# satoken/ractip

Hardware: AMD Instinct MI355X
Metric: sequence-pairs/sec (incl. bp+hp+ap DP; host strings in, thresholded matrices out) at n=500 (higher is better)
Workload: dtype f64; 1 GPU; synthetic random pairs n=500/500, std::mt19937(12345) stream (BASELINE config 3); scoring=CONTRAfold complementary (708 weights)

## Files before the change

### ractip_amd/csrc/compute.hip

```cpp
#include <hip/hip_runtime.h>

#include <algorithm>
#include <cmath>
#include <cstring>
#include <string>
#include <vector>

#include "ctx.h"
#include "kernels.h"

namespace rh::host {

template <class L, class... Args>
int run_graphed(rh_ctx* c, GraphSlot& g, hipStream_t stream, int k, L launcher, const Args&... args)
{
    const auto launch = [&] { int rc = RH_OK; ((rc = rc ? rc : launcher(c, args)), ...); return rc; };
    if (!c->use_graphs || c->time_cls >= 0) return launch();
    size_t key = 1469598103934665603ull + (sizeof(Args) + ...);
    const auto mix = [&](const void* p, size_t n) { for (size_t q = 0; q < n; q++) key = (key ^ ((const unsigned char*)p)[q]) * 0x100000001b3ull; };
    (mix(&args, sizeof(Args)), ...);
    int *launch_counter = &c->n_launch[k], *far_counter = &c->n_far[k];
    if (!g.exec || g.key != key) {
        if (g.exec) { HIP_TRY(c, hipGraphExecDestroy(g.exec)); g.exec = nullptr; }
        hipGraph_t graph = nullptr;
        const int before = *launch_counter, far_before = *far_counter;
        HIP_TRY(c, hipStreamBeginCapture(stream, hipStreamCaptureModeThreadLocal));
        const int rc = launch();
        hipError_t e = hipStreamEndCapture(stream, &graph);
        if (rc) { if (graph) (void)hipGraphDestroy(graph); return rc; }
        if (e != hipSuccess) { if (graph) (void)hipGraphDestroy(graph); return fail(c, RH_ERR_HIP, "graph capture failed: %s", hipGetErrorString(e)); }
        e = hipGraphInstantiate(&g.exec, graph, nullptr, nullptr, 0);
        (void)hipGraphDestroy(graph);
        if (e != hipSuccess) { g.exec = nullptr; return fail(c, RH_ERR_HIP, "hipGraphInstantiate failed: %s", hipGetErrorString(e)); }
        g.key = key;
        g.launches = *launch_counter - before;
        g.far = *far_counter - far_before;
        *launch_counter = before;
        *far_counter = far_before;
    }
    HIP_TRY(c, hipGraphLaunch(g.exec, stream));
    *launch_counter += g.launches;
    *far_counter += g.far;
    return RH_OK;
}

McLinArgs mc_lin_args(const rh_ctx* c, int phase, const McBatch& B, const LinSet* lin, bool routed)
{
    McLinArgs A;
    A.B = B; A.lin = lin; A.phase = phase;
    A.logz = c->d_mclogz.as<double>(); A.bad = c->d_bad.as<int>();
    A.plan = plan_mc_lin(c, phase, B.nmax);
    if (routed && (!c->small_list.empty() || c->n_short > 0)) {
        A.routed = 1;
        A.small_list = c->d_small_list.as<const int>(); A.n_small = (int)c->small_list.size();
        A.n_sweep = c->d_n_sweep.as<const int>(); A.nmax_sweep = c->nmax_sweep;
        A.n_short = c->d_n_short.as<const int>(); A.nmax_short = c->nmax_short; A.short_count = c->n_short;
        A.plan_sweep = plan_mc_lin(c, phase, A.nmax_sweep);
        A.plan_short = plan_mc_lin(c, phase, A.nmax_short);
    }
    A.pin = xcd_pin(B.ns);
    A.strip_xcd = c->strip_xcd;
    A.f5_jlo = 32;
    A.f5_pass = c->f5_pass && f5_pass_lds(B.ld, 1) <= 64 * 1024;
    return A;
}

static McVlinArgs mc_vlin_args(const rh_ctx* c, int phase, bool co)
{
    McVlinArgs A;
    A.B = co ? c->co : c->mc; A.phase = phase; A.co = co;
    A.pin = xcd_pin(A.B.ns);
    A.plan = plan_mc_vlin(c, phase, co, A.B.nmax);
    A.d_vlin = c->d_vlin; A.h_vlin = c->h_vlin; A.hplen = c->h_hplen.data(); A.d_hplen = c->d_hplen.as<const double>();
    A.bad = co ? c->d_cobad.as<int>() : c->d_bad.as<int>();
    if (co) {
        const DxBatch& D = c->dx;
        if (A.B.seeded) { A.from = c->mc; A.pair_seq = c->d_pidx.as<const int>(); }
        A.hp = D.hp; A.hp_logz = D.logz; A.hp_stride = D.tab_stride; A.hp_ldd = D.ldd; A.n1max = D.n1max; A.n2max = D.n2max;
        A.cut_min = c->co_cut_min; A.cut_max = c->co_cut_max;
        A.window = c->co_window && c->co_cut_min >= 1 && (phase == 1 || A.B.seeded);
    } else {
        A.logz = c->d_mclogz.as<double>(); A.gaps = c->d_gaps.as<double>(); A.max_w = c->max_w;
        A.acc_wide = c->acc_wide && (size_t)VM_COUNT * A.B.tab_stride * sizeof(double) < ((size_t)1 << 32);
        A.acc_final_t = c->acc_final_t && c->max_w <= 15;
    }
    return A;
}

static DxLinArgs dx_args(const rh_ctx* c)
{
    DxLinArgs A;
    A.X = c->dxl; A.plan = c->plan[2]; A.lz_chunks = c->lz_chunks;
    A.zpart = c->d_zpart.as<double>(); A.zbar = c->d_zbar.as<double>();
    A.logz = c->d_logz.as<double>(); A.bad = c->d_dxbad.as<int>();
    return A;
}

DxLinArgs dx_lin_args(const rh_ctx* c)
{
    DxLinArgs A = dx_args(c);
    A.dm = c->d_dxlin; A.hm = &c->h_dxlin;
    return A;
}

static DxLinArgs dx_vlin_args(const rh_ctx* c)
{
    DxLinArgs A = dx_args(c);
    A.vdx_s = c->vdx_s; A.sem20 = c->vienna_sem == kViennaSem20;
    return A;
}

int flagged(rh_ctx* c, const int* d_flags, int n, hipStream_t st, std::vector<int>* set)
{
    std::vector<int> flags(n);
    HIP_TRY(c, hipMemcpyAsync(flags.data(), d_flags, sizeof(int) * n, hipMemcpyDeviceToHost, st));
    HIP_TRY(c, hipStreamSynchronize(st));
    set->clear();
    for (int k = 0; k < n; k++) if (flags[k]) set->push_back(k);
    return RH_OK;
}

struct Attempt {
    bool defer_log = false;
    bool deferred = false;
    std::vector<int> flagged_seqs;
    std::vector<int> flagged_pairs;
    bool went_log = false;
    Ev outside_from = kEvMcInside;
};

static int close_dx_phase(rh_ctx* c)
{
    HIP_TRY(c, hipEventRecord(c->ev[kEvDxEnd], c->s_dx));
    if (!c->overlap) HIP_TRY(c, hipStreamSynchronize(c->s_dx));
    return RH_OK;
}

template <class Launch>
static int restart_mc_log(rh_ctx* c, Launch launch)
{
    c->n_launch[0] = c->n_launch[1] = 0;
    c->n_far[0] = c->n_far[1] = 0;
    HIP_TRY(c, hipEventRecord(c->ev[kEvMcStart], c->s_mc));
    HIP_TRY(c, hipMemsetAsync(c->d_bp.p, 0, sizeof(double) * c->mc.tri_stride * c->mc.ns, c->s_mc));
    if (int rc = launch()) return rc;
    if (c->last_path == 0) c->last_path = 2;
// ... 280 lines not shown
```

### ractip_amd/csrc/ctx.h

```cpp
#pragma once
#include <hip/hip_runtime.h>

#include <cassert>
#include <cstdint>
#include <cstring>
#include <string>
#include <type_traits>
#include <vector>

#include "../../include/ractip_hot.h"
#include "batch.h"
#include "score_model.h"
#include "lin_model.h"
#include "vienna_model.h"
#include "scale_order.h"

struct rh_ctx;

namespace rh::host {

struct DevBuf {
    void* p = nullptr;
    size_t cap = 0;
    DevBuf() = default;
// ... 248 lines not shown
    McBatch co = {};
    DevBuf d_coseq;
    DevBuf d_con;
    DevBuf d_cotab;
    DevBuf d_cof5;
    DevBuf d_cobp;
    DevBuf d_cobad;
    double ms[4] = {0, 0, 0, 0};
    int n_launch[3] = {0, 0, 0};
    int n_far[3] = {0, 0, 0};
    bool overlap = true;
    int time_cls = -1;
    std::vector<hipEvent_t> tev;
    size_t tev_n = 0;
    Ctx() = default;
    Ctx(const Ctx&) = delete;
    ~Ctx() { delete[] lin_r; delete h_score; delete h_vienna; }
};

}

struct rh_ctx : rh::host::Ctx {};

#define HIP_TRY(c, call)                                                                         \
    do {                                                                                         \
        hipError_t e_ = (call);                                                                  \
        if (e_ != hipSuccess)                                                                    \
            return fail(c, e_ == hipErrorOutOfMemory ? RH_ERR_OOM : RH_ERR_HIP, "%s failed: %s", \
                        #call, hipGetErrorString(e_));                                           \
    } while (0)

#define KLAUNCH(c, cls, kern, grid, block, stream, ...)                                                   \
    do {                                                                                                  \
        const bool timed_ = (c)->time_cls == (cls) && (c)->tev_n + 2 <= (c)->tev.size();                  \
        if (timed_) (void)hipEventRecord((c)->tev[(c)->tev_n++], stream);                                 \
        hipLaunchKernelGGL(kern, grid, block, 0, stream, __VA_ARGS__);                                    \
        if (timed_) (void)hipEventRecord((c)->tev[(c)->tev_n++], stream);                                 \
    } while (0)

namespace rh::host {

inline size_t tri_size(int n) { return (size_t)(n + 1) * (n + 2) / 2; }

int fail(rh_ctx* c, int code, const char* fmt, ...);
int ensure(rh_ctx* c, DevBuf& buf, size_t bytes, bool zero);
int stage(rh_ctx* c, int ns, const char* const* seqs, const int* lens, bool with_mc, bool with_dx, const char* const* cons = nullptr,
          const char* const* co_cons = nullptr, int npairs = 0, const int* first = nullptr, const int* second = nullptr);
inline int seq_of(const Ctx* c, int p, int side) { return c->pair_seq[2 * (size_t)p + side]; }
inline void pairs_of_seq(const Ctx* c, int k, std::vector<int>* pairs)
{
    for (int p = 0; p < c->np; p++)
        if (seq_of(c, p, 0) == k || seq_of(c, p, 1) == k) pairs->push_back(p);
}
template <class K> struct Named { K kern; const char* name; };
#define NAMED(...) {__VA_ARGS__, #__VA_ARGS__}
template <class Row, size_t N, class Pred>
const Row& row_of(const Row (&rows)[N], Pred&& is)
{
    for (const Row& r : rows) if (is(r)) return r;
    assert(!"the plan names a kernel combination that has no row");
    return rows[0];
}
inline int xcd_pin(int ns) { return ns % 8 == 0 ? 1 : 0; }
inline dim3 seq_grid(int pin, int ns, int groups) { return pin ? dim3(ns, groups) : dim3(groups, ns); }
struct SweepPass {
    rh_ctx* c;
    const SweepPlan& P;
    const McBatch& B;
    hipStream_t st;
    int k;
    int far2_next = -1;
    int last_block() const { return P.BS > 0 ? (B.nmax - 1) / P.BS : 0; }
};
int launch_mc_log(rh_ctx* c, int pin, const McBatch& B, double* logz_out);
SweepPlan plan_mc_lin(const rh_ctx* c, int phase, int nmax);
int launch_mc_lin(rh_ctx* c, const McLinArgs& A);
void far_products(const rh_ctx* c, int phase, int nmax, bool mfma, SweepPlan* P);
const char* far_name(SweepPlan::Far far, int BS, int phase);
void far_inside_after(const SweepPass& S, int done);
void far_outside_begin(SweepPass& S, int top);
void far_outside_before(SweepPass& S, int d);
std::vector<double> strip_weights(const LinModel& L, bool* ok_out = nullptr);
size_t f5_pass_lds(int ld, int phase);
int launch_mc_vienna(rh_ctx* c, int pin);
SweepPlan plan_mc_vlin(const rh_ctx* c, int phase, bool co, int nmax);
int launch_mc_vlin(rh_ctx* c, const McVlinArgs& A);
int launch_cofold(rh_ctx* c);
int select_vlin(rh_ctx* c, int model);
extern const double kVRungS[Ctx::kVRungs];
int launch_dx_log(rh_ctx* c, const DxBatch& D);
SweepPlan plan_dx_lin(const rh_ctx* c, int w);
SweepPlan plan_dx_vlin(bool sem20);
int launch_dx_lin(rh_ctx* c, const DxLinArgs& A);
int launch_dx_vlin(rh_ctx* c, const DxLinArgs& A);
int launch_dx_vlog(rh_ctx* c);
int retry_mc_lin_rungs(rh_ctx* c, int first_model, std::vector<int>* rest, int (&rescued_by)[Ctx::kRungs + 1]);
int recompute_mc_subset_log(rh_ctx* c, const std::vector<int>& F);
int retry_dx_lin_rungs(rh_ctx* c, std::vector<int>* rest);
int recompute_dx_subset_log(rh_ctx* c, const std::vector<int>& F);
int recompute_pairs_on_helper(rh_ctx* c, const std::vector<int>& P);
int compute(rh_ctx* c);
McLinArgs mc_lin_args(const rh_ctx* c, int phase, const McBatch& B, const LinSet* lin, bool routed);
DxLinArgs dx_lin_args(const rh_ctx* c);
int flagged(rh_ctx* c, const int* d_flags, int n, hipStream_t st, std::vector<int>* set);

}

rh_ctx* make_ctx_for_helper(int device, int model, const char* param_file, const char* defaults_file, int use_bl, int semantics);
```

### ractip_amd/csrc/launch_contrafold.hip

```cpp
#include <hip/hip_runtime.h>

#include <algorithm>
#include <cmath>
#include <cstring>
#include <string>
#include <vector>

#include "ctx.h"
#include "kernels.h"

__global__ void log_finish(rh::McBatch B, double* __restrict__ logz)
{
    const int sq = blockIdx.x * blockDim.x + threadIdx.x;
    if (sq < B.ns) logz[sq] = B.f5i[(size_t)sq * B.ld + B.n[sq]];
}

namespace rh::host {

int launch_mc_log(rh_ctx* c, int pin, const McBatch& B, double* logz_out)
{
    hipLaunchKernelGGL(mc_init, dim3((B.ns + 63) / 64), dim3(64), 0, c->s_mc, B);
    for (int d = 0; d <= B.nmax - 1; d++) {
        const int waves = std::max(B.nmax - 1 - d, 0) + 1;
        KLAUNCH(c, 0, mc_inside_diag, pin ? dim3(B.ns, (waves + 3) / 4) : dim3((waves + 3) / 4, B.ns), dim3(256), c->s_mc, B, c->d_model, d, pin);
        c->n_launch[0]++;
    }
    HIP_TRY(c, hipEventRecord(c->ev[kEvMcInside], c->s_mc));
    for (int d = B.nmax - 2; d >= 0; d--) {
        const int waves = (B.nmax - 1 - d) + 1;
        KLAUNCH(c, 2, mc_outside_diag, pin ? dim3(B.ns, (waves + 3) / 4) : dim3((waves + 3) / 4, B.ns), dim3(256), c->s_mc, B, c->d_model, d, pin);
        c->n_launch[1]++;
    }
    hipLaunchKernelGGL(log_finish, dim3((B.ns + 63) / 64), dim3(64), 0, c->s_mc, B, logz_out);
    hipLaunchKernelGGL(mc_unpaired, dim3((B.nmax + 63) / 64, B.ns), dim3(256), 0, c->s_mc, B);
    return RH_OK;
}

using InsideDiagK = void (*)(McBatch, const LinModel*, int, double, int);
struct DiagKernels { int W, BS; Named<InsideDiagK> in; Named<decltype(&lin_outside_diag<4, 16>)> out; };
#define DIAG(W, BS) {W, BS, NAMED(lin_inside_diag<W, BS, 0>), NAMED(lin_outside_diag<W, BS>)}
const DiagKernels kDiag[] = {DIAG(8, 0), DIAG(16, 0), DIAG(4, 16), DIAG(8, 16), DIAG(16, 16), DIAG(8, 32), DIAG(16, 32)};
const Named<InsideDiagK> kInsidePair = NAMED(lin_inside_diag<4, 16, 3>);
const Named<InsideDiagK> kInsideAhead[2] = {NAMED(lin_inside_diag<4, 16, 1>), NAMED(lin_inside_diag<4, 16, 2>)};
struct PairKernels { int W; Named<decltype(&lin_outside_pair<4, 16>)> out; };
const PairKernels kOutsidePair[] = {{4, NAMED(lin_outside_pair<4, 16>)}, {8, NAMED(lin_outside_pair<8, 16>)}};
struct StripKernels { int W, filt; Named<decltype(&lin_inside_strip<8, 4, 0>)> in; Named<decltype(&lin_outside_strip<8, 4, 0>)> out; };
#define STRIP(W, FILT) {W, FILT, NAMED(lin_inside_strip<8, W, FILT>), NAMED(lin_outside_strip<8, W, FILT>)}
const StripKernels kStrip[] = {STRIP(4, 0), STRIP(8, 1), STRIP(8, 0)};
struct LdsKernels { int BS; Named<decltype(&lin_far_inside<16>)> in, out; };
const LdsKernels kLds[] = {{16, NAMED(lin_far_inside<16>), NAMED(lin_far_outside<16>)}, {32, NAMED(lin_far_inside<32>), NAMED(lin_far_outside<32>)}};
const Named<decltype(&lin_far_inside_mfma)> kFarGather[2] = {NAMED(lin_far_inside_mfma), NAMED(lin_far_outside_mfma)};
const Named<decltype(&lin_far_inside_pk)> kFarPacked[2] = {NAMED(lin_far_inside_pk), NAMED(lin_far_outside_pk)};
#undef DIAG
#undef STRIP
static const DiagKernels& diag_kernels(int W, int BS) { return row_of(kDiag, [&](const DiagKernels& r) { return r.W == W && r.BS == BS; }); }
static const PairKernels& pair_kernels(int W) { return row_of(kOutsidePair, [&](const PairKernels& r) { return r.W == W; }); }
static const StripKernels& strip_kernels(int W, int filt) { return row_of(kStrip, [&](const StripKernels& r) { return r.W == W && r.filt == filt; }); }
static const LdsKernels& lds_kernels(int BS) { return row_of(kLds, [&](const LdsKernels& r) { return r.BS == BS; }); }

const char* far_name(SweepPlan::Far far, int BS, int phase)
{
    switch (far) {
        case SweepPlan::kFarLds: return phase == 0 ? lds_kernels(BS).in.name : lds_kernels(BS).out.name;
        case SweepPlan::kFarGather: return kFarGather[phase].name;
        case SweepPlan::kFarPacked: return kFarPacked[phase].name;
        default: return "";
    }
}
void far_products(const rh_ctx* c, int phase, int nmax, bool mfma, SweepPlan* P)
{
    const int from = c->far2 >= 0 ? (c->far2 ? 1 : 0) : 384;
    P->far = P->BS == 0 ? SweepPlan::kFarNone : !mfma ? SweepPlan::kFarLds : c->far_pk ? SweepPlan::kFarPacked : SweepPlan::kFarGather;
    P->far2_from = P->far == SweepPlan::kFarPacked && from > 0 && nmax >= from ? from : 0;
    P->far_name = far_name(P->far, P->BS, phase);
}

void far_inside_after(const SweepPass& S, int done)
{
    rh_ctx* c = S.c;
    const McBatch& B = S.B;
    const int D = S.P.BS ? done / S.P.BS + 1 : 0, last_block = S.last_block(), l2 = S.P.far2_from;
    if (S.P.BS == 0 || done % S.P.BS != 0 || D < 4 || D > last_block) return;
    if (S.P.far == SweepPlan::kFarLds) KLAUNCH(c, 1, (lds_kernels(S.P.BS).in.kern), dim3(last_block - D + 1, B.ns), dim3(256), S.st, B, D);
    else if (S.P.far == SweepPlan::kFarGather) KLAUNCH(c, 1, (kFarGather[0].kern), dim3(last_block - D + 1, B.ns), dim3(256), S.st, B, D);
    else {
        KLAUNCH(c, 1, lin_pack_tiles<0>, dim3(B.nb - (D - 2), B.ns, 2), dim3(256), S.st, B, D - 2, 0, (int)S.P.banded);
        if (l2 && (D + 3) % 4 == 0) {
            const int D2 = (D + 3) / 4, last2 = (B.nmax - 1) / 64;
            if (D2 >= 4 && D2 <= last2) KLAUNCH(c, 1, lin_far2_inside, dim3(last2 - D2 + 1, B.ns), dim3(256), S.st, B, D2, l2);
        }
        KLAUNCH(c, 1, (kFarPacked[0].kern), dim3(last_block - D + 1, B.ns), dim3(256), S.st, B, D, l2);
// ... 1 lines not shown
    c->n_launch[S.k]++;
    c->n_far[S.k]++;
}
void far_outside_before(SweepPass& S, int d)
{
    rh_ctx* c = S.c;
    const McBatch& B = S.B;
    const int D = S.P.BS ? (d + 1) / S.P.BS - 1 : 0, last_block = S.last_block(), l2 = S.P.far2_from;
    if (S.P.BS == 0 || (d + 1) % S.P.BS != 0 || D < 0 || D > last_block) return;
    if (S.P.far == SweepPlan::kFarLds) KLAUNCH(c, 3, (lds_kernels(S.P.BS).out.kern), dim3(last_block - D + 1, B.ns, 2), dim3(256), S.st, B, D);
    else if (S.P.far == SweepPlan::kFarGather) KLAUNCH(c, 3, (kFarGather[1].kern), dim3(last_block - D + 1, B.ns, 2), dim3(256), S.st, B, D);
    else {
        if (D + 2 <= last_block) KLAUNCH(c, 3, lin_pack_tiles<1>, dim3(B.nb - (D + 2), B.ns, 1), dim3(256), S.st, B, D + 2, 1, 0);
        if (l2) {
            const int last2 = (B.nmax - 1) / 64;
            for (; S.far2_next >= 0 && 4 * S.far2_next + 3 >= D; S.far2_next--)
                KLAUNCH(c, 3, lin_far2_outside, dim3(last2 - S.far2_next + 1, B.ns, 2), dim3(256), S.st, B, S.far2_next, l2);
        }
        KLAUNCH(c, 3, (kFarPacked[1].kern), dim3(last_block - D + 1, B.ns, 2), dim3(256), S.st, B, D, l2);
    }
    c->n_launch[S.k]++;
    c->n_far[S.k]++;
}
void far_outside_begin(SweepPass& S, int top)
{
    if (S.P.BS == 0) return;
    rh_ctx* c = S.c;
    const McBatch& B = S.B;
    const int last_block = S.last_block(), banded = S.P.banded;
    if (S.P.far == SweepPlan::kFarPacked) {
        S.far2_next = (B.nmax - 1) / 64;
        if (S.P.repack2 && last_block - 1 > 2) KLAUNCH(c, 3, lin_pack_tiles<1>, dim3(B.nb - 2, B.ns, 2), dim3(256), S.st, B, 2, 0, banded);
        for (int Dblk = std::max(2, last_block - 1); Dblk <= last_block; Dblk++)
            KLAUNCH(c, 3, lin_pack_tiles<1>, dim3(B.nb - Dblk, B.ns, 2), dim3(256), S.st, B, Dblk, 0, banded);
    }
    for (int d = (last_block + 1) * S.P.BS - 1; d > top; d -= S.P.BS) far_outside_before(S, d);
}

SweepPlan plan_mc_lin(const rh_ctx* c, int phase, int nmax)
{
    SweepPlan P;
    const int w = phase == 0 ? c->lin_w_in : c->lin_w;
    P.BS = c->lin_bs == 0 || c->lin_bs == 32 ? c->lin_bs : 16;
    P.W = w == 16 ? 16 : (w == 4 && P.BS == 16 ? 4 : 8);
    const bool all_orgs = P.W == 4 && P.BS == 16, strips_ok = c->far_pk && c->far_mfma && c->lin_bs == 16 && nmax >= kStripMinN;
    const bool strips_on = (c->strip & (phase == 0 ? 1 : 2)) && strips_ok, strips = all_orgs && strips_on;
    const StripKernels& strip = strip_kernels(c->strip_w, c->strip_w == 8 && c->strip_filt && c->strip_filt_ok);
    const DiagKernels& diag = diag_kernels(P.W, P.BS);
    bool mfma = P.BS == 16 && c->far_mfma;
    P.org = SweepPlan::kDiagonals;
    P.fine = phase == 0 ? diag.in.name : diag.out.name;
    if (strips) {
        P.org = SweepPlan::kStrips;
        P.W = strip.W;
        P.filt = strip.filt;
    } else if (phase == 0 && all_orgs && c->lookahead == 2) {
        P.org = SweepPlan::kPairs;
        P.fine = kInsidePair.name;
        mfma = true;
    } else if (phase == 0 && all_orgs && c->lookahead) {
        P.org = SweepPlan::kLookahead;
        P.fine = kInsideAhead[0].name;
    } else if (phase == 1 && mfma && (P.W == 4 || P.W == 8) && c->lookahead == 2) {
        P.org = SweepPlan::kPairs;
        P.fine = pair_kernels(P.W).out.name;
    }
    far_products(c, phase, nmax, mfma, &P);
    P.banded = strips;
    P.repack2 = phase == 1 && strips != (all_orgs && (c->strip & 1) && strips_ok);
    if (strips_on) P.fine = phase == 0 ? strip.in.name : strip.out.name;
    if (phase == 0 && P.org == SweepPlan::kPairs && !c->far_mfma) { P.fine = diag.in.name; P.far_name = far_name(SweepPlan::kFarLds, 16, 0); }
    return P;
}

static void inside_pairs(const SweepPass& S, const McLinArgs& A, int last)
{
    for (int d = 0; d <= last; d += 2) {
        const int groups = (std::max(S.B.nmax - 1 - d, 0) + 62) / 63 + 1;
        KLAUNCH(S.c, 0, (kInsidePair.kern), seq_grid(A.pin, S.B.ns, groups), dim3(256), S.st, S.B, A.lin->d, d, std::exp(-A.lin->h.s * d), A.pin);
        S.c->n_launch[0]++;
        far_inside_after(S, d + 2);
    }
}
size_t f5_pass_lds(int ld, int phase) { return sizeof(double) * ((size_t)ld + 8 + (phase ? (size_t)((ld + 255) / 256) * 256 : 0)); }

static void inside_strips(const SweepPass& S, const McLinArgs& A)
{
    rh_ctx* c = S.c;
    const McBatch& B = S.B;
    constexpr int KD = 8, GS = 64 - (KD - 1);
    const auto strip = strip_kernels(S.P.W, S.P.filt).in.kern;
    inside_pairs(S, A, 30);
    for (int d0 = 32; d0 <= B.nmax - 2; d0 += KD) {
        const int groups = (B.nmax - 1 - d0 + GS - 1) / GS;
        KLAUNCH(c, 0, strip, seq_grid(A.pin, B.ns, groups), dim3(64 * S.P.W), S.st, B, A.lin->d, A.lin->wT, d0, std::exp(-A.lin->h.s * d0),
                (A.pin && A.strip_xcd) ? 2 : A.pin);
        c->n_launch[0]++;
        far_inside_after(S, d0 + KD);
    }
    if (A.f5_pass) hipLaunchKernelGGL(lin_f5i_pass, dim3(B.ns), dim3(256), f5_pass_lds(B.ld, 0), S.st, B, A.lin->d, A.f5_jlo);
    else hipLaunchKernelGGL(lin_f5i_tail, dim3(B.ns), dim3(256), 0, S.st, B, A.lin->d, A.f5_jlo);
}
static void inside_diagonals(const SweepPass& S, const McLinArgs& A, bool ahead)
{
    const InsideDiagK full = diag_kernels(S.P.W, S.P.BS).in.kern;
    for (int d = 0; d <= S.B.nmax - 1; d++) {
        const int groups = (std::max(S.B.nmax - 1 - d, 0) + 63) / 64 + 1;
        const bool odd = ahead && (d & 1);
        KLAUNCH(S.c, 0, (!ahead ? full : kInsideAhead[odd].kern), seq_grid(A.pin, S.B.ns, groups), dim3(odd ? 64 : 64 * S.P.W), S.st, S.B, A.lin->d, d,
                std::exp(-A.lin->h.s * d), A.pin);
        S.c->n_launch[0]++;
        far_inside_after(S, d + 1);
    }
}

static void outside_strips(SweepPass& S, const McLinArgs& A)
{
    rh_ctx* c = S.c;
    const McBatch& B = S.B;
    constexpr int KD = 8, GS = 64 - (KD - 1);
    const auto strip = strip_kernels(S.P.W, S.P.filt).out.kern;
    const int d0_top = (B.nmax - 2) | (KD - 1);
    far_outside_begin(S, d0_top);
    if (A.f5_pass) hipLaunchKernelGGL(lin_f5o_pass, dim3(B.ns), dim3(256), f5_pass_lds(B.ld, 1), S.st, B, A.lin->d);
    else hipLaunchKernelGGL(lin_f5o_head, dim3(B.ns), dim3(256), 0, S.st, B, A.lin->d, B.nmax - 1, 1);
    for (int d0 = d0_top; d0 >= KD - 1; d0 -= KD) {
        far_outside_before(S, d0);
        const int groups = (B.nmax - 1 - (d0 - (KD - 1)) + GS - 1) / GS;
        KLAUNCH(c, 2, strip, seq_grid(A.pin, B.ns, groups), dim3(64 * S.P.W), S.st, B, A.lin->d, A.lin->wT, d0, (A.pin && A.strip_xcd) ? 2 : A.pin, A.bad);
        c->n_launch[1]++;
    }
}
static void outside_pairs(SweepPass& S, const McLinArgs& A)
{
    const auto pair = pair_kernels(S.P.W).out.kern;
    far_outside_begin(S, S.B.nmax - 2);
    for (int d = (S.B.nmax - 2) | 1; d >= 0; d -= 2) {
        for (int r = d; r >= d - 1 && r >= 0; r--) far_outside_before(S, r);
        const int ncol = S.B.nmax - 1 - d + 1;
        const int groups = std::max(1, (ncol - 1 + 62) / 63) + 1;
        KLAUNCH(S.c, 2, pair, seq_grid(A.pin, S.B.ns, groups), dim3(64 * S.P.W), S.st, S.B, A.lin->d, d, d, A.pin, A.bad);
        S.c->n_launch[1]++;
    }
}
static void outside_diagonals(SweepPass& S, const McLinArgs& A)
{
    const auto diag = diag_kernels(S.P.W, S.P.BS).out.kern;
    far_outside_begin(S, S.B.nmax - 2);
    for (int d = S.B.nmax - 2; d >= 0; d--) {
        far_outside_before(S, d);
        const int groups = (S.B.nmax - 1 - d + 63) / 64 + 1;
        KLAUNCH(S.c, 2, diag, seq_grid(A.pin, S.B.ns, groups), dim3(64 * S.P.W), S.st, S.B, A.lin->d, d, A.pin, A.bad);
        S.c->n_launch[1]++;
    }
}

int launch_mc_lin(rh_ctx* c, const McLinArgs& A)
{
    const McBatch& BR = A.B;
    const int phase = A.phase;
    const auto sweep = [&](const McBatch& B, const SweepPlan& Q) {
        SweepPass S{c, Q, B, c->s_mc, phase};
        if (Q.org == SweepPlan::kStrips) return phase == 0 ? inside_strips(S, A) : outside_strips(S, A);
        if (Q.org == SweepPlan::kPairs) return phase == 0 ? inside_pairs(S, A, B.nmax) : outside_pairs(S, A);
        return phase == 0 ? inside_diagonals(S, A, Q.org == SweepPlan::kLookahead) : outside_diagonals(S, A);
    };
    if (phase == 0) {
// ... 70 lines not shown
```

### ractip_amd/csrc/mccaskill_strip.hip

```cpp
#include <hip/hip_runtime.h>

#include <type_traits>
#include <utility>

#include "batch.h"
#include "dev_util.h"
#include "lin_model.h"
#include "kernels.h"

namespace rh {

namespace {

template <int V> using IC = std::integral_constant<int, V>;
template <class F, int... Is> __device__ __forceinline__ void static_for_impl(F&& f, std::integer_sequence<int, Is...>) { (f(IC<Is>{}), ...); }
template <int N, class F> __device__ __forceinline__ void static_for(F&& f) { static_for_impl(f, std::make_integer_sequence<int, N>{}); }

}

#ifdef RH_STAMPS
__device__ unsigned long long g_stamps[16];
#define RH_STAMP(k) do { const unsigned long long t_ = __builtin_amdgcn_s_memtime(); st_acc_[k] += t_ - t_prev_; t_prev_ = t_; \
        if ((k) == 8 && threadIdx.x == 0) { for (int k_ = 0; k_ < 15; k_++) if (st_acc_[k_]) atomicAdd(&g_stamps[k_], st_acc_[k_]); atomicAdd(&g_stamps[15], 1ull); } } while (0)
#define RH_STAMP_BEGIN() unsigned long long st_acc_[15] = {}; unsigned long long t_prev_ = __builtin_amdgcn_s_memtime()
extern "C" int rh_debug_stamps(unsigned long long* out, int reset)
{
    if (hipMemcpyFromSymbol(out, HIP_SYMBOL(g_stamps), sizeof(g_stamps)) != hipSuccess) return -1;
    if (reset) { unsigned long long z[16] = {}; if (hipMemcpyToSymbol(HIP_SYMBOL(g_stamps), z, sizeof(z)) != hipSuccess) return -1; }
    return 0;
}
__device__ unsigned long long g_trace[5 * 16384];
extern "C" int rh_debug_trace(unsigned long long* out)
{
    return hipMemcpyFromSymbol(out, HIP_SYMBOL(g_trace), sizeof(g_trace)) == hipSuccess ? 0 : -1;
}
#if RH_STAMPS == 3
#define RH_TRACE(slot) do { if (threadIdx.x == 0 && d0 == 256) { const unsigned lin_ = blockIdx.x + blockIdx.y * gridDim.x; if (lin_ < 16384) g_trace[5 * lin_ + (slot)] = __builtin_amdgcn_s_memrealtime(); } } while (0)
#define RH_TRACE_ID() do { if (threadIdx.x == 0 && d0 == 256) { const unsigned lin_ = blockIdx.x + blockIdx.y * gridDim.x; if (lin_ < 16384) g_trace[5 * lin_] = ((unsigned long long)__builtin_amdgcn_s_getreg((20 << 0) | (0 << 6) | (31 << 11)) << 32) | __builtin_amdgcn_s_getreg((4 << 0) | (0 << 6) | (31 << 11)); } } while (0)
#endif
#define RH_NOSTAMP(k) do { } while (0)
#define RH_NOSTAMP_BEGIN() do { } while (0)
#if RH_STAMPS == 3
#define RH_STAMPO(k) RH_NOSTAMP(k)
#define RH_STAMPO_BEGIN() RH_NOSTAMP_BEGIN()
#define RH_STAMPI(k) RH_NOSTAMP(k)
#define RH_STAMPI_BEGIN() RH_NOSTAMP_BEGIN()
#elif RH_STAMPS == 2
#define RH_STAMPO(k) RH_STAMP(k)
#define RH_STAMPO_BEGIN() RH_STAMP_BEGIN()
#define RH_STAMPI(k) RH_NOSTAMP(k)
#define RH_STAMPI_BEGIN() RH_NOSTAMP_BEGIN()
#else
#define RH_STAMPI(k) RH_STAMP(k)
#define RH_STAMPI_BEGIN() RH_STAMP_BEGIN()
#define RH_STAMPO(k) RH_NOSTAMP(k)
#define RH_STAMPO_BEGIN() RH_NOSTAMP_BEGIN()
#endif
#else
#define RH_STAMPI(k) do { } while (0)
#define RH_STAMPI_BEGIN() do { } while (0)
#define RH_STAMPO(k) do { } while (0)
#define RH_STAMPO_BEGIN() do { } while (0)
#endif
#ifndef RH_TRACE
#define RH_TRACE(slot) do { } while (0)
#define RH_TRACE_ID() do { } while (0)
#endif

template <int U, bool OUTSIDE, int CE>
__device__ __forceinline__ void filt_factored(lds_vp xb, lds_vp fw, const double* __restrict__ F, double (&g)[4])
{
    auto X = [&](int row_off, int m, int l1) -> double { return OUTSIDE ? xb[row_off + 31 + m - l1] : xb[row_off + 3 - m + l1]; };
    constexpr int par = (U + 1) & 1;
    double bw[15];
#pragma unroll
    for (int j = 0; j < 15; j++) bw[j] = F[160 + 16 * par + j];
    static_for<8>([&](auto QC) {
        constexpr int q = decltype(QC)::value, t0 = U - 1 + 4 * q, ro = q * 4 * CE;
        if constexpr (t0 + 6 >= 2 && t0 <= 30) {
            double S = 0.0, xc = 0.0;
            if constexpr (t0 >= 3) {
                double S2 = 0.0;
                static_for<t0 - 1>([&](auto LC) {
                    constexpr int l1 = decltype(LC)::value + 1, dist = (2 * l1 - t0) < 0 ? (t0 - 2 * l1) : (2 * l1 - t0);
                    if constexpr (2 * l1 != t0) {
                        const double x = X(ro, 0, l1);
                        if constexpr (l1 & 1) S = fma(bw[dist / 2], x, S); else S2 = fma(bw[dist / 2], x, S2);
                    }
                });
// ... 468 lines not shown
        fm2s[SL] = fm2; gs[SL] += g0 + g1;
    };
    auto fin = [&](auto KC) {
        constexpr int K = decltype(KC)::value, SL = K / W;
        const int d = d0 + K;
        const bool v = i <= n - 1 - d;
        double fm2 = fm2s[SL];
        const double g = gs[SL];
        if constexpr (K >= 1) {
            fm2 = fma(f1[0], SFM[(K - 1) * CS + lane + 1], fm2);
            if (1 <= d - 32) fm2 = fma(SFM1[(K - 1) * CS + lane], LDm[lane + K], fm2);
        }
        double x01 = p_x01, x10 = p_x10, x11 = p_x11, o_fc = p_fc, o_fca = p_fca, o_fm1 = p_fm1, o_fm = p_fm;
        if constexpr (K >= 3) { x01 = SFCX[(K - 3) * CS + lane + 1]; x10 = SFCX[(K - 3) * CS + lane + 2]; }
        if constexpr (K >= 4) x11 = SFCX[(K - 4) * CS + lane + 2];
        if constexpr (K >= 2) { o_fc = SFC[(K - 2) * CS + lane + 1]; o_fca = SFCA[(K - 2) * CS + lane + 1]; }
        if constexpr (K >= 1) { o_fm1 = SFM1[(K - 1) * CS + lane + 1]; o_fm = SFM[(K - 1) * CS + lane]; }
        double lk = lam_d0;
#pragma unroll
        for (int q = 0; q < K; q++) lk *= lam;
        const double hp = lk * hp30;
        const double sp = p_c01[SL] * x01 + p_c10[SL] * x10 + p_c11[SL] * x11;
        double fc = p_tjb[SL] * (g + sp + hp) + p_cst[SL] * o_fc + fm2 * p_ctja[SL];
        double fm1v = o_fca * w_mp2 + o_fm1 * w_mu;
        double fmv = fm2 + o_fm * w_mu + fm1v;
        if (!v) { fc = 0.0; fm1v = 0.0; fmv = 0.0; }
        const double fcxv = fc * p_cbx[SL], fcav = fc * p_cba[SL];
        SFM[K * CS + lane] = fmv; SFM1[K * CS + lane] = fm1v; SFCX[K * CS + lane] = fcxv; SFC[K * CS + lane] = fc; SFCA[K * CS + lane] = fcav;
    };
    RH_STAMPI(6);
#define RH_SLOT(T)                                                                                  \
    if constexpr (T < KD) {                                                                         \
        if (w == T % W) fin(IC<T>{});                                                               \
        if constexpr (T >= 1 && T + 1 < KD)                                                         \
            static_for<KD>([&](auto KC) {                                                           \
                constexpr int K = decltype(KC)::value;                                              \
                if constexpr (K > T) { if (w == K % W) addrow(IC<(T >= 1 ? T - 1 : 0)>{}, KC); }    \
            });                                                                                     \
        if constexpr (T + 1 < KD) lds_barrier();                                                    \
    }
    RH_SLOT(0) RH_SLOT(1) RH_SLOT(2) RH_SLOT(3) RH_SLOT(4) RH_SLOT(5) RH_SLOT(6) RH_SLOT(7)
#undef RH_SLOT
    RH_STAMPI(7);
    lds_barrier();
    if (lane < GS) {
#pragma unroll 1
        for (int r = w; r < 5 * KD; r += W) {
            const int tb = r / KD, k = r - tb * KD, d = d0 + k;
            const int slot_of[5] = {L_FM, L_FM1, L_FCX, L_FC, L_FCA};
            if (i <= n - 1 - d) tab[slot_of[tb] * ts + (size_t)d * ld + i] = SFM[r * CS + lane];
        }
    }
    RH_STAMPI(8);
    RH_TRACE(4);
}

__device__ __forceinline__ double f5_term(double f5, double fca, double acc) { return fma(f5, fca, acc); }
__device__ __forceinline__ double f5_entry(double prev, double r0, double r1, double r2, double r3, double w_eu, double w_ep2)
{
    return fma(prev, w_eu, (r0 + r1 + r2 + r3) * w_ep2);
}

__global__ __launch_bounds__(256) void lin_f5i_tail(McBatch B, const LinModel* __restrict__ L, int jlo)
{
    __shared__ double red[4];
    const int sq = blockIdx.x;
    if (sq >= B.ns) return;
    const int n = B.n[sq], ld = B.ld;
    const int w = threadIdx.x >> 6, lane = threadIdx.x & 63;
    double* __restrict__ f5i = B.f5i + (size_t)sq * ld;
    const double* __restrict__ fca = B.tab + (size_t)sq * B.seq_stride + L_FCA * B.tab_stride;
#pragma unroll 1
    for (int jj = jlo < 1 ? 1 : jlo; jj <= n; jj++) {
        double acc = 0.0;
        for (int k = threadIdx.x; k <= jj - 2; k += 256) acc = f5_term(f5i[k], fca[(size_t)(jj - 2 - k) * ld + (k + 1)], acc);
        acc = wsum(acc);
        if (lane == 0) red[w] = acc;
        __syncthreads();
        if (threadIdx.x == 0) f5i[jj] = f5_entry(f5i[jj - 1], red[0], red[1], red[2], red[3], L->w_eu, L->w_ep2);
        __syncthreads();
    }
}

constexpr int kF5Blk = 16;

__global__ __launch_bounds__(256) void lin_f5i_pass(McBatch B, const LinModel* __restrict__ L, int jlo)
{
    extern __shared__ double f5_lds[];
    const int sq = blockIdx.x;
    if (sq >= B.ns) return;
    const int n = B.n[sq], ld = B.ld;
    if (n < jlo) return;
    const int t = threadIdx.x, w = t >> 6, lane = t & 63;
    double* const f5s = f5_lds;
    double* const red = f5_lds + ld;
    double* __restrict__ f5i = B.f5i + (size_t)sq * ld;
    const double* __restrict__ fca = B.tab + (size_t)sq * B.seq_stride + L_FCA * B.tab_stride;
    const double w_eu = L->w_eu, w_ep2 = L->w_ep2;
    for (int k = t; k < jlo; k += 256) f5s[k] = f5i[k];
    __syncthreads();
    double prev = f5s[jlo - 1];
#pragma unroll 1
    for (int jj0 = jlo; jj0 <= n; jj0 += kF5Blk) {
        const int ne = n - jj0 + 1 < kF5Blk ? n - jj0 + 1 : kF5Blk;
        const int kmax = jj0 + ne - 3;
        double acc[kF5Blk], opin[kF5Blk];
#pragma unroll
        for (int e = 0; e < kF5Blk; e++) { acc[e] = 0.0; opin[e] = 0.0; }
        int kin = 0x7fffffff;
        auto fetch = [&](int k, double (&op)[kF5Blk]) {
            const int kc = k <= kmax ? k : kmax;
            const double* __restrict__ col = fca + (kc + 1);
#pragma unroll
            for (int e = 0; e < kF5Blk; e++) {
                const int row = jj0 + (e < ne ? e : 0) - 2 - kc;
                op[e] = col[(size_t)(row > 0 ? row : 0) * ld];
            }
        };
        auto take = [&](int k, const double (&op)[kF5Blk]) {
            if (k > kmax) return;
            if (k < jj0) {
                const double f = f5s[k];
#pragma unroll
                for (int e = 0; e < kF5Blk; e++) acc[e] = (e < ne && (e > 0 || k <= jj0 - 2)) ? f5_term(f, op[e], acc[e]) : acc[e];
            } else {
                kin = k;
#pragma unroll
                for (int e = 2; e < kF5Blk; e++) opin[e] = op[e];
            }
        };
#pragma unroll 1
        for (int k = t; k <= kmax; k += 512) {
            double opa[kF5Blk], opb[kF5Blk];
            fetch(k, opa);
            fetch(k + 256, opb);
            take(k, opa);
            take(k + 256, opb);
        }
#pragma unroll
        for (int e = 0; e < kF5Blk; e++) {
            if (e < ne) {
                const int jj = jj0 + e;
                double a = acc[e];
                if (e >= 2 && kin <= jj - 2) a = f5_term(f5s[kin], opin[e], a);
                a = wsum(a);
                if (lane == 0) red[(e & 1) * 4 + w] = a;
                lds_barrier();
                const double* r = red + (e & 1) * 4;
                prev = f5_entry(prev, r[0], r[1], r[2], r[3], w_eu, w_ep2);
                if (t == 0) f5s[jj] = prev;
            }
        }
        lds_barrier();
        if (t < ne) f5i[jj0 + t] = f5s[jj0 + t];
    }
}

template <int KD, int W>
struct OutStripPlan {
    static constexpr int GS = 64 - (KD - 1);
    static constexpr int NM = 31;
    static constexpr int TS = 4;
    static constexpr int RD = NM + KD, CD = 72;
    static constexpr int RA = NM + KD, CA = 96;
    static constexpr int RE = 32, CE = 96;
    static constexpr int OFF_DUMMY = RD * CD + RA * CA + RE * CE;
    static constexpr int SZ = OFF_DUMMY + CA + 320;
    static constexpr int PADL = 8, CS = 72;
    static constexpr int KEEP = (KD - 1) * CD;
    static constexpr int OFF_PART = KEEP;
    static constexpr int OFF_S = OFF_PART + TS * KD * 3 * 64;
    static_assert(OFF_S + 5 * KD * CS <= SZ, "overlay does not fit");
    static_assert(SZ * 8 <= 80 * 1024, "two workgroups per CU");
};

__global__ __launch_bounds__(256) void lin_f5o_head(McBatch B, const LinModel* __restrict__ L, int khi, int klo)
{
    __shared__ double red[4];
    const int sq = blockIdx.x;
    if (sq >= B.ns) return;
    const int n = B.n[sq], ld = B.ld;
    const int w = threadIdx.x >> 6, lane = threadIdx.x & 63;
    const double* __restrict__ fca_tab = B.tab + (size_t)sq * B.seq_stride + L_FCA * B.tab_stride;
    double* __restrict__ f5o = B.f5o + (size_t)sq * ld;
#pragma unroll 1
    for (int k = khi; k >= klo && k >= 1; k--) {
        if (k > n - 1) continue;
        const double* __restrict__ fca = fca_tab + (k + 1);
        double acc = 0.0;
        for (int jj = k + 2 + threadIdx.x; jj <= n; jj += 256) acc = f5_term(f5o[jj], fca[(size_t)(jj - 2 - k) * ld], acc);
        acc = wsum(acc);
        if (lane == 0) red[w] = acc;
        __syncthreads();
        if (threadIdx.x == 0) f5o[k] = f5_entry(f5o[k + 1], red[0], red[1], red[2], red[3], L->w_eu, L->w_ep2);
        __syncthreads();
    }
}

__global__ __launch_bounds__(256) void lin_f5o_pass(McBatch B, const LinModel* __restrict__ L)
{
    extern __shared__ double f5_lds[];
    const int sq = blockIdx.x;
    if (sq >= B.ns) return;
    const int n = B.n[sq], ld = B.ld;
    if (n < 2) return;
    const int t = threadIdx.x, w = t >> 6, lane = t & 63;
    double* const f5s = f5_lds;
    double* const red = f5_lds + ld;
    double* const park = red + 8;
    const double* __restrict__ fca = B.tab + (size_t)sq * B.seq_stride + L_FCA * B.tab_stride;
    double* __restrict__ f5o = B.f5o + (size_t)sq * ld;
    const double w_eu = L->w_eu, w_ep2 = L->w_ep2;
    double prev = f5o[n];
    if (t == 0) f5s[n] = prev;
    __syncthreads();
#pragma unroll 1
    for (int k0 = n - 1; k0 >= 1; k0 -= kF5Blk) {
        const int ne = k0 < kF5Blk ? k0 : kF5Blk;
        const int rmax = n - 2 - (k0 - ne + 1);
        double acc[kF5Blk];
#pragma unroll
        for (int e = 0; e < kF5Blk; e++) acc[e] = 0.0;
        auto fetch = [&](int r, double (&op)[kF5Blk]) {
            const double* __restrict__ row = fca + (size_t)(r <= rmax ? r : 0) * ld;
#pragma unroll
            for (int e = 0; e < kF5Blk; e++) op[e] = row[k0 - (e < ne ? e : 0) + 1];
        };
        auto take = [&](int q, int r, const double (&op)[kF5Blk]) {
            if (r > rmax) return;
#pragma unroll
            for (int e = 0; e < kF5Blk; e++) {
                if (e >= 2 && t <= e - 2) park[(q * kF5Blk + e) * 16 + t] = op[e];
                else if (e < ne && k0 - e + 2 + r <= n) acc[e] = f5_term(f5s[k0 - e + 2 + r], op[e], acc[e]);
            }
        };
#pragma unroll 1
        for (int q = 0; t + 256 * q <= rmax; q += 2) {
            double opa[kF5Blk], opb[kF5Blk];
            fetch(t + 256 * q, opa);
            fetch(t + 256 * q + 256, opb);
            take(q, t + 256 * q, opa);
            take(q + 1, t + 256 * q + 256, opb);
        }
#pragma unroll
        for (int e = 0; e < kF5Blk; e++) {
            if (e < ne) {
                const int k = k0 - e;
                double a = acc[e];
                if (e >= 2 && t <= e - 2) {
                    a = 0.0;
                    for (int q = 0; k + 2 + t + 256 * q <= n; q++) a = f5_term(f5s[k + 2 + t + 256 * q], park[(q * kF5Blk + e) * 16 + t], a);
                }
                a = wsum(a);
                if (lane == 0) red[(e & 1) * 4 + w] = a;
                lds_barrier();
                const double* r = red + (e & 1) * 4;
                prev = f5_entry(prev, r[0], r[1], r[2], r[3], w_eu, w_ep2);
                if (t == 0) f5s[k] = prev;
            }
        }
        lds_barrier();
        if (t < ne) f5o[k0 - t] = f5s[k0 - t];
    }
}

template <int KD, int W, int FILT>
__global__ __launch_bounds__(64 * W, (W >= 8 ? 4 : 2)) void lin_outside_strip(McBatch B, const LinModel* __restrict__ L, const double* __restrict__ wT, int d0,
                                                                              int pin, int* __restrict__ bad)
{
    using P = OutStripPlan<KD, W>;
    constexpr int GS = P::GS, NM = P::NM, CD = P::CD, CA = P::CA, CE = P::CE, CS = P::CS, PADL = P::PADL;
    constexpr int NSL = KD / W;
    constexpr int TS = P::TS, KH = KD * TS / W;
    static_assert(KD % W == 0 && KD <= 8 && W % TS == 0 && KD % (W / TS) == 0 && (NM + 1) % W == 0, "8 terms per end and term set, 32/W staged rows per wavefront and region");
    __shared__ double lds[P::SZ];
    constexpr bool FACT = FILT != 0 && W == 8 && KD == 8;
    __shared__ double fw[FACT ? 160 : 1];
    int sq = pin ? blockIdx.x : blockIdx.y, slot = pin ? blockIdx.y : blockIdx.x;
    if (pin == 2) {
        const unsigned lin = blockIdx.x + blockIdx.y * gridDim.x, t = lin >> 3;
        slot = (int)(t % gridDim.y);
        sq = (int)(t / gridDim.y) * 8 + (int)(lin & 7);
    }
    if (sq >= B.ns) return;
    const int n = B.n[sq];
    const int w = __builtin_amdgcn_readfirstlane(threadIdx.x >> 6), lane = threadIdx.x & 63;
    const int wt = w % TS, kb = (w / TS) * KH;
    const int ld = B.ld;
    const size_t ts = B.tab_stride;
    const uint8_t* __restrict__ s = B.seq + (size_t)sq * B.lds;
    double* __restrict__ tab = B.tab + (size_t)sq * B.seq_stride;
    const double* __restrict__ f5i = B.f5i + (size_t)sq * ld;
    double* __restrict__ f5o = B.f5o + (size_t)sq * ld;
    const int dlow = d0 - (KD - 1);
    const int ncell_max = n - 1 - dlow > 0 ? n - 1 - dlow : 0;
    const int ngroup = (ncell_max + GS - 1) / GS;
    if (slot >= ngroup) return;

#ifdef RH_STAGGER
    {
        const unsigned lin = blockIdx.x + blockIdx.y * gridDim.x;
        if (lin >= 256 && lin < 512) for (int q = 0; q < RH_STAGGER; q++) __builtin_amdgcn_s_sleep(127);
    }
#endif
    RH_STAMPO_BEGIN();
    const int i0 = 1 + slot * GS - (KD - 1);
    const int i = i0 + lane;
    double* const LDm = lds;
    double* const LA = lds + P::RD * CD;
    double* const LE = LA + P::RA * CA;
    const double* __restrict__ fm = tab + L_FM * ts;
    const double* __restrict__ fm1 = tab + L_FM1 * ts;
    const double* __restrict__ fm2o = tab + L_FM2O * ts;
    const double* __restrict__ fcox = tab + L_FCOX * ts;

    int s_j[NSL], s_jp1[NSL], s_jp2[NSL];
    int s_im1, s_i, s_ip1;
    int rb0, rb1, rb2, r0[NSL], r1[NSL], r2[NSL];
    {
        const int top = B.lds - 1;
        const int c_i = i < 1 ? 1 : (i < top ? i : top - 1);
        rb0 = s[c_i - 1]; rb1 = s[c_i]; rb2 = s[c_i + 1];
#pragma unroll
        for (int sl = 0; sl < NSL; sl++) {
            const int j = i + d0 - (w + W * sl), cj = j < 0 ? 0 : (j + 2 <= top ? j : top - 2);
            r0[sl] = s[cj]; r1[sl] = s[cj + 1]; r2[sl] = s[cj + 2];
        }
    }

    constexpr int NR = (NM + 1) / W;
    constexpr int NT = (NM + 1) / TS;
    static_assert(NR % 2 == 0 && NR <= 8, "row tails are paired");
    double vA0[NR], vA1[NR / 2], vD0[NR], vD1, vE0[NR], vE1[NR / 2], a_lo[NT], a_hi[NT];
    const int lhalf = lane >> 5, lsub = lane & 31;
// ... 441 lines not shown
```

Measured before the change: 12290 pairs/s.

## Stage f5 pass operands through LDS with software-pipelined chunked global loads

Rewrites the lin_f5i_pass and lin_f5o_pass kernels so the fca operand tiles are loaded cooperatively, 16 entries per row across threads, into a padded LDS staging buffer. The next chunk's global loads are issued while the current chunk is consumed. This is meant to replace scattered strided per-thread global loads with coalesced loads and to hide latency. The park buffer is compacted and launch bounds are raised to 4 blocks per CU to leave room for staging. The cost is more barriers per chunk and extra LDS use, and the pass is now gated on the staging area fitting.

```diff
diff --git a/ractip_amd/csrc/compute.hip b/ractip_amd/csrc/compute.hip
--- a/ractip_amd/csrc/compute.hip
+++ b/ractip_amd/csrc/compute.hip
@@ -61,7 +61,7 @@
     A.pin = xcd_pin(B.ns);
     A.strip_xcd = c->strip_xcd;
     A.f5_jlo = 32;
-    A.f5_pass = c->f5_pass && f5_pass_lds(B.ld, 1) <= 64 * 1024;
+    A.f5_pass = c->f5_pass && f5_pass_fits(B.ld);
     return A;
 }
 
diff --git a/ractip_amd/csrc/ctx.h b/ractip_amd/csrc/ctx.h
--- a/ractip_amd/csrc/ctx.h
+++ b/ractip_amd/csrc/ctx.h
@@ -354,6 +354,7 @@
 void far_outside_before(SweepPass& S, int d);
 std::vector<double> strip_weights(const LinModel& L, bool* ok_out = nullptr);
 size_t f5_pass_lds(int ld, int phase);
+bool f5_pass_fits(int ld);
 int launch_mc_vienna(rh_ctx* c, int pin);
 SweepPlan plan_mc_vlin(const rh_ctx* c, int phase, bool co, int nmax);
 int launch_mc_vlin(rh_ctx* c, const McVlinArgs& A);
diff --git a/ractip_amd/csrc/f5_stage.h b/ractip_amd/csrc/f5_stage.h
--- /dev/null
+++ b/ractip_amd/csrc/f5_stage.h
@@ -0,0 +1,52 @@
+#pragma once
+#include <stddef.h>
+
+#if defined(__HIPCC__)
+#define RH_F5_HD __host__ __device__ inline
+#else
+#define RH_F5_HD inline
+#endif
+
+namespace rh {
+
+constexpr int kF5Blk = 16;
+constexpr int kF5Threads = 256;
+constexpr int kF5StageRows = 128;
+constexpr int kF5StageRowsMin = 32;
+constexpr int kF5StageStride = 17;
+constexpr int kF5StageLoads = kF5StageRows * kF5Blk / kF5Threads;
+constexpr int kF5ParkT = 14;
+constexpr int kF5LdsDoubles = 64 * 1024 / 8;
+
+RH_F5_HD int f5_park_slot(int q, int e, int t) { return (q * kF5ParkT + (e - 2)) * kF5ParkT + t; }
+RH_F5_HD int f5_fixed_doubles(int ld, int phase) { return ld + 8 + (phase ? (ld + 255) / 256 * kF5ParkT * kF5ParkT : 0); }
+RH_F5_HD int f5_stage_rows(int ld, int phase)
+{
+    const int room = (kF5LdsDoubles - f5_fixed_doubles(ld, phase)) / kF5StageStride;
+    return room >= kF5StageRows ? kF5StageRows : room < 0 ? 0 : room & ~(kF5Threads / kF5Blk - 1);
+}
+RH_F5_HD int f5_lds_doubles(int ld, int phase) { return f5_fixed_doubles(ld, phase) + f5_stage_rows(ld, phase) * kF5StageStride; }
+
+RH_F5_HD int f5_chunks(int top, int R) { return top < 0 ? 0 : top / R + 1; }
+struct F5Chunk { int lo, hi; };
+RH_F5_HD F5Chunk f5o_chunk(int top, int R, int c) { return F5Chunk{c * R, c * R + R - 1 < top ? c * R + R - 1 : top}; }
+RH_F5_HD F5Chunk f5i_chunk(int top, int R, int c) { return f5o_chunk(top, R, f5_chunks(top, R) - 1 - c); }
+
+RH_F5_HD int f5_stage_row(int t, int i) { return (t >> 4) + (kF5Threads / kF5Blk) * i; }
+RH_F5_HD int f5_stage_entry(int t) { return t & (kF5Blk - 1); }
+RH_F5_HD int f5_stage_slot(int row_in_chunk, int e) { return row_in_chunk * kF5StageStride + e; }
+
+RH_F5_HD int f5o_last_row(int n, int k0, int ne, int e) { return e < ne ? n - 2 - k0 + e : -1; }
+RH_F5_HD size_t f5o_addr(int ld, int k0, int r, int e) { return (size_t)r * ld + (k0 + 1 - e); }
+RH_F5_HD int f5o_owned_row(int lo, int t) { return lo + ((t - lo) & (kF5Threads - 1)); }
+
+RH_F5_HD int f5i_term(int jj0, int d, int e) { return jj0 + e - 2 - d; }
+RH_F5_HD int f5i_last_row(int jj0, int ne, int e) { return e < ne ? jj0 + e - 2 : -1; }
+RH_F5_HD size_t f5i_addr(int ld, int jj0, int d, int e) { return (size_t)d * ld + (jj0 - 1 - d + e); }
+RH_F5_HD int f5i_owned_term(int jj0, int hi, int e, int t)
+{
+    const int klo = f5i_term(jj0, hi, e);
+    return klo + ((t - klo) & (kF5Threads - 1));
+}
+
+}
diff --git a/ractip_amd/csrc/launch_contrafold.hip b/ractip_amd/csrc/launch_contrafold.hip
--- a/ractip_amd/csrc/launch_contrafold.hip
+++ b/ractip_amd/csrc/launch_contrafold.hip
@@ -7,6 +7,7 @@
 #include <vector>
 
 #include "ctx.h"
+#include "f5_stage.h"
 #include "kernels.h"
 
 __global__ void log_finish(rh::McBatch B, double* __restrict__ logz)
@@ -174,7 +175,8 @@
         far_inside_after(S, d + 2);
     }
 }
-size_t f5_pass_lds(int ld, int phase) { return sizeof(double) * ((size_t)ld + 8 + (phase ? (size_t)((ld + 255) / 256) * 256 : 0)); }
+size_t f5_pass_lds(int ld, int phase) { return sizeof(double) * (size_t)f5_lds_doubles(ld, phase); }
+bool f5_pass_fits(int ld) { return f5_stage_rows(ld, 1) >= kF5StageRowsMin; }
 
 static void inside_strips(const SweepPass& S, const McLinArgs& A)
 {
diff --git a/ractip_amd/csrc/mccaskill_strip.hip b/ractip_amd/csrc/mccaskill_strip.hip
--- a/ractip_amd/csrc/mccaskill_strip.hip
+++ b/ractip_amd/csrc/mccaskill_strip.hip
@@ -5,6 +5,7 @@
 
 #include "batch.h"
 #include "dev_util.h"
+#include "f5_stage.h"
 #include "lin_model.h"
 #include "kernels.h"
 
@@ -639,9 +640,25 @@
     }
 }
 
-constexpr int kF5Blk = 16;
-
-__global__ __launch_bounds__(256) void lin_f5i_pass(McBatch B, const LinModel* __restrict__ L, int jlo)
+
+__device__ __forceinline__ void f5_stage_issue(const double* __restrict__ fca, const double* __restrict__ cell, ptrdiff_t step, int t, int lo, int last,
+                                               double (&v)[kF5StageLoads])
+{
+#pragma unroll
+    for (int i = 0; i < kF5StageLoads; i++) {
+        const int row = lo + f5_stage_row(t, i);
+        const double* __restrict__ p = cell + row * step;
+        v[i] = *(row <= last ? p : fca + 1);
+    }
+}
+__device__ __forceinline__ void f5_stage_store(double* stg, int t, int R, const double (&v)[kF5StageLoads])
+{
+#pragma unroll
+    for (int i = 0; i < kF5StageLoads; i++)
+        if (kF5Blk * i < R) stg[f5_stage_slot(f5_stage_row(t, i), f5_stage_entry(t))] = v[i];
+}
+
+__global__ __launch_bounds__(256, 4) void lin_f5i_pass(McBatch B, const LinModel* __restrict__ L, int jlo)
 {
     extern __shared__ double f5_lds[];
     const int sq = blockIdx.x;
@@ -649,57 +666,65 @@
     const int n = B.n[sq], ld = B.ld;
     if (n < jlo) return;
     const int t = threadIdx.x, w = t >> 6, lane = t & 63;
+    const int R = f5_stage_rows(ld, 0);
     double* const f5s = f5_lds;
     double* const red = f5_lds + ld;
+    double* const stg = f5_lds + f5_fixed_doubles(ld, 0);
     double* __restrict__ f5i = B.f5i + (size_t)sq * ld;
     const double* __restrict__ fca = B.tab + (size_t)sq * B.seq_stride + L_FCA * B.tab_stride;
     const double w_eu = L->w_eu, w_ep2 = L->w_ep2;
     for (int k = t; k < jlo; k += 256) f5s[k] = f5i[k];
     __syncthreads();
     double prev = f5s[jlo - 1];
+    double v[kF5StageLoads];
+    const auto issue = [&](int jj0, int c, double (&v)[kF5StageLoads]) {
+        const int ne = n - jj0 + 1 < kF5Blk ? n - jj0 + 1 : kF5Blk, e = f5_stage_entry(t), dmax = f5i_last_row(jj0, ne, e);
+        const F5Chunk ch = f5i_chunk(jj0 + ne - 3, R, c);
+        f5_stage_issue(fca, fca + f5i_addr(ld, jj0, 0, e), (ptrdiff_t)f5i_addr(ld, jj0, 1, 0) - (ptrdiff_t)f5i_addr(ld, jj0, 0, 0), t, ch.lo, dmax < ch.hi ? dmax : ch.hi, v);
+    };
 #pragma unroll 1
-    for (int jj0 = jlo; jj0 <= n; jj0 += kF5Blk) {
+    for (int jb = jlo; jb <= n; jb += kF5Blk) {
+        const int jj0 = __builtin_amdgcn_readfirstlane(jb);
         const int ne = n - jj0 + 1 < kF5Blk ? n - jj0 + 1 : kF5Blk;
-        const int kmax = jj0 + ne - 3;
-        double acc[kF5Blk], opin[kF5Blk];
-#pragma unroll
-        for (int e = 0; e < kF5Blk; e++) { acc[e] = 0.0; opin[e] = 0.0; }
+        const int top = jj0 + ne - 3;
+        double acc[kF5Blk];
+#pragma unroll
+        for (int e = 0; e < kF5Blk; e++) acc[e] = 0.0;
         int kin = 0x7fffffff;
-        auto fetch = [&](int k, double (&op)[kF5Blk]) {
-            const int kc = k <= kmax ? k : kmax;
-            const double* __restrict__ col = fca + (kc + 1);
-#pragma unroll
-            for (int e = 0; e < kF5Blk; e++) {
-                const int row = jj0 + (e < ne ? e : 0) - 2 - kc;
-                op[e] = col[(size_t)(row > 0 ? row : 0) * ld];
-            }
-        };
-        auto take = [&](int k, const double (&op)[kF5Blk]) {
-            if (k > kmax) return;
-            if (k < jj0) {
-                const double f = f5s[k];
-#pragma unroll
-                for (int e = 0; e < kF5Blk; e++) acc[e] = (e < ne && (e > 0 || k <= jj0 - 2)) ? f5_term(f, op[e], acc[e]) : acc[e];
-            } else {
-                kin = k;
-#pragma unroll
-                for (int e = 2; e < kF5Blk; e++) opin[e] = op[e];
-            }
-        };
+        const int nc = f5_chunks(top, R);
+        issue(jj0, 0, v);
 #pragma unroll 1
-        for (int k = t; k <= kmax; k += 512) {
-            double opa[kF5Blk], opb[kF5Blk];
-            fetch(k, opa);
-            fetch(k + 256, opb);
-            take(k, opa);
-            take(k + 256, opb);
+        for (int c = 0; c < nc; c++) {
+            const F5Chunk ch = f5i_chunk(top, R, c);
+            f5_stage_store(stg, t, R, v);
+            lds_barrier();
+            if (c + 1 < nc) issue(jj0, c + 1, v);
+            lds_vp vstg = (lds_vp)stg, vf5 = (lds_vp)f5s;
+#pragma unroll
+            for (int e0 = 0; e0 < kF5Blk; e0 += 4) {
+                double op[4], f[4];
+                bool ex[4];
+#pragma unroll
+                for (int u = 0; u < 4; u++) {
+                    const int e = e0 + u, k = f5i_owned_term(jj0, ch.hi, e, t), d = f5i_term(jj0, k, e);
+                    const bool own = e < ne && k >= 0 && d >= ch.lo;
+                    ex[u] = own && k < jj0;
+                    kin = own && k >= jj0 ? k : kin;
+                    op[u] = vstg[f5_stage_slot(own ? d - ch.lo : 0, e)];
+                    f[u] = vf5[ex[u] ? k : 0];
+                }
+#pragma unroll
+                for (int u = 0; u < 4; u++) acc[e0 + u] = ex[u] ? f5_term(f[u], op[u], acc[e0 + u]) : acc[e0 + u];
+                asm volatile("" : "+v"(acc[e0]), "+v"(acc[e0 + 1]), "+v"(acc[e0 + 2]), "+v"(acc[e0 + 3]));
+            }
+            if (c + 1 < nc) lds_barrier();
         }
 #pragma unroll
         for (int e = 0; e < kF5Blk; e++) {
             if (e < ne) {
                 const int jj = jj0 + e;
                 double a = acc[e];
-                if (e >= 2 && kin <= jj - 2) a = f5_term(f5s[kin], opin[e], a);
+                if (e >= 2 && kin <= jj - 2) a = f5_term(f5s[kin], stg[f5_stage_slot(f5i_term(jj0, kin, e), e)], a);
                 a = wsum(a);
                 if (lane == 0) red[(e & 1) * 4 + w] = a;
                 lds_barrier();
@@ -754,7 +779,7 @@
     }
 }
 
-__global__ __launch_bounds__(256) void lin_f5o_pass(McBatch B, const LinModel* __restrict__ L)
+__global__ __launch_bounds__(256, 4) void lin_f5o_pass(McBatch B, const LinModel* __restrict__ L)
 {
     extern __shared__ double f5_lds[];
     const int sq = blockIdx.x;
@@ -762,42 +787,67 @@
     const int n = B.n[sq], ld = B.ld;
     if (n < 2) return;
     const int t = threadIdx.x, w = t >> 6, lane = t & 63;
+    const int R = f5_stage_rows(ld, 1);
     double* const f5s = f5_lds;
     double* const red = f5_lds + ld;
     double* const park = red + 8;
+    double* const stg = f5_lds + f5_fixed_doubles(ld, 1);
     const double* __restrict__ fca = B.tab + (size_t)sq * B.seq_stride + L_FCA * B.tab_stride;
     double* __restrict__ f5o = B.f5o + (size_t)sq * ld;
     const double w_eu = L->w_eu, w_ep2 = L->w_ep2;
     double prev = f5o[n];
     if (t == 0) f5s[n] = prev;
     __syncthreads();
+    double v[kF5StageLoads];
+    const auto issue = [&](int k0, int c, double (&v)[kF5StageLoads]) {
+        const int ne = k0 < kF5Blk ? k0 : kF5Blk, e = f5_stage_entry(t), rlast = f5o_last_row(n, k0, ne, e);
+        const F5Chunk ch = f5o_chunk(n - 2 - (k0 - ne + 1), R, c);
+        f5_stage_issue(fca, fca + f5o_addr(ld, k0, 0, e), ld, t, ch.lo, rlast < ch.hi ? rlast : ch.hi, v);
+    };
 #pragma unroll 1
-    for (int k0 = n - 1; k0 >= 1; k0 -= kF5Blk) {
+    for (int kb = n - 1; kb >= 1; kb -= kF5Blk) {
+        const int k0 = __builtin_amdgcn_readfirstlane(kb);
         const int ne = k0 < kF5Blk ? k0 : kF5Blk;
         const int rmax = n - 2 - (k0 - ne + 1);
         double acc[kF5Blk];
 #pragma unroll
         for (int e = 0; e < kF5Blk; e++) acc[e] = 0.0;
-        auto fetch = [&](int r, double (&op)[kF5Blk]) {
-            const double* __restrict__ row = fca + (size_t)(r <= rmax ? r : 0) * ld;
-#pragma unroll
-            for (int e = 0; e < kF5Blk; e++) op[e] = row[k0 - (e < ne ? e : 0) + 1];
-        };
-        auto take = [&](int q, int r, const double (&op)[kF5Blk]) {
-            if (r > rmax) return;
-#pragma unroll
-            for (int e = 0; e < kF5Blk; e++) {
-                if (e >= 2 && t <= e - 2) park[(q * kF5Blk + e) * 16 + t] = op[e];
-                else if (e < ne && k0 - e + 2 + r <= n) acc[e] = f5_term(f5s[k0 - e + 2 + r], op[e], acc[e]);
-            }
-        };
+        const auto exists = [&](int r, int e) { return r <= f5o_last_row(n, k0, ne, e); };
+        const int nc = f5_chunks(rmax, R);
+        issue(k0, 0, v);
 #pragma unroll 1
-        for (int q = 0; t + 256 * q <= rmax; q += 2) {
-            double opa[kF5Blk], opb[kF5Blk];
-            fetch(t + 256 * q, opa);
-            fetch(t + 256 * q + 256, opb);
-            take(q, t + 256 * q, opa);
-            take(q + 1, t + 256 * q + 256, opb);
+        for (int c = 0; c < nc; c++) {
+            const F5Chunk ch = f5o_chunk(rmax, R, c);
+            f5_stage_store(stg, t, R, v);
+            lds_barrier();
+            if (c + 1 < nc) issue(k0, c + 1, v);
+            const int r = f5o_owned_row(ch.lo, t), q = r >> 8;
+            if (r <= ch.hi) {
+                const double* const row = stg + f5_stage_slot(r - ch.lo, 0);
+                lds_vp vrow = (lds_vp)row, vf5 = (lds_vp)f5s;
+#pragma unroll
+                for (int e0 = 0; e0 < kF5Blk; e0 += 4) {
+                    double op[4], f[4];
+#pragma unroll
+                    for (int u = 0; u < 4; u++) {
+                        const int jj = k0 - (e0 + u) + 2 + r;
+                        op[u] = vrow[e0 + u];
+                        f[u] = vf5[jj <= n ? jj : n];
+                    }
+#pragma unroll
+                    for (int u = 0; u < 4; u++) {
+                        const int e = e0 + u;
+                        acc[e] = (exists(r, e) && !(e >= 2 && t <= e - 2)) ? f5_term(f[u], op[u], acc[e]) : acc[e];
+                    }
+                    asm volatile("" : "+v"(acc[e0]), "+v"(acc[e0 + 1]), "+v"(acc[e0 + 2]), "+v"(acc[e0 + 3]));
+                }
+                if (t < kF5ParkT) {
+#pragma unroll
+                    for (int e = 2; e < kF5Blk; e++)
+                        if (t <= e - 2 && exists(r, e)) park[f5_park_slot(q, e, t)] = row[e];
+                }
+            }
+            lds_barrier();
         }
 #pragma unroll
         for (int e = 0; e < kF5Blk; e++) {
@@ -806,7 +856,7 @@
                 double a = acc[e];
                 if (e >= 2 && t <= e - 2) {
                     a = 0.0;
-                    for (int q = 0; k + 2 + t + 256 * q <= n; q++) a = f5_term(f5s[k + 2 + t + 256 * q], park[(q * kF5Blk + e) * 16 + t], a);
+                    for (int q = 0; k + 2 + t + 256 * q <= n; q++) a = f5_term(f5s[k + 2 + t + 256 * q], park[f5_park_slot(q, e, t)], a);
                 }
                 a = wsum(a);
                 if (lane == 0) red[(e & 1) * 4 + w] = a;
```

After: 12500 pairs/s, median of 6. 1.02x the previous value.
